# Sreyan88/audio-ssl

Measured on AMD Instinct MI355X. Metric: upstream clips/sec (1s@16kHz, 64-mel), higher is better.
Workload: dtype bf16; 1 GPU; delores-m upstream step (log-mel + 2 views + q/k conv encoders + MoCo + 3 Barlow heads + bwd + SGD), 1 s @ 16 kHz, 64 mel, batch 512/GPU, queue 65536; global_batch=512, parallelism=dp1

## Files before the change

### audio-ssl_amd/csrc/conv.hip

```cpp
#include <cstdlib>
#include "common.h"

namespace {

constexpr int CH = 64, KTOT = 576;
constexpr int WPITCH = KTOT + 8;
constexpr int PIXP = 72;
constexpr int PIXW = 96;

typedef __attribute__((address_space(3))) bf16x4* lds4_t;

struct ConvArgs {
    const bf16* X; const bf16* W; const float* bias; bf16* Y; double* sum; double* sumsq;
    int Ti, rows_total, tiles, out_f32, dbg, stat_rep;
    const float* gamma; bf16* Praw;
};

template <int FI, int PITCH, int NTH = 256>
struct Halo {
    static constexpr int TT = 256 / FI;
    static constexpr int COLS = FI + 2;
    static constexpr int ELEMS = (TT + 2) * COLS * PITCH;
    static constexpr int NV = ((TT + 2) * FI * 8 + NTH - 1) / NTH;
    static constexpr int NVEC = (TT + 2) * FI * 8;
// ... 410 lines not shown
#pragma unroll
                    for (int j = 0; j < 4; ++j) {
                        const unsigned d0 = q[0][j] ^ sm[j], d1 = q[1][j] ^ sm[j], d2 = q[2][j] ^ sm[j], d3 = q[3][j] ^ sm[j];
                        const float hi = vmax4(__builtin_bit_cast(float, d0), __builtin_bit_cast(float, d1),
                                               __builtin_bit_cast(float, d2), __builtin_bit_cast(float, d3));
                        const float lo = vmax4(__builtin_bit_cast(float, d0 << 16), __builtin_bit_cast(float, d1 << 16),
                                               __builtin_bit_cast(float, d2 << 16), __builtin_bit_cast(float, d3 << 16));
                        r[j] = __builtin_amdgcn_perm(__builtin_bit_cast(unsigned, hi), __builtin_bit_cast(unsigned, lo), 0x07060302u) ^ sm[j];
                    }
                    const unsigned odd = 0u - (unsigned)(pl & 1);
                    r = u32x4{(r[2] & odd) | (r[0] & ~odd), (r[3] & odd) | (r[1] & ~odd), (r[0] & odd) | (r[2] & ~odd), (r[1] & odd) | (r[3] & ~odd)};
                    if (a.rows_total - grow >= 2)
                        *reinterpret_cast<u32x4*>(reinterpret_cast<char*>(a.Praw) + ((grow >> 1) * (FI / 2) * 128 + po * 128 + cp * 16)) = r;
                }
            }
        }
        if (ts) ts[tsi++] = __builtin_amdgcn_s_memtime();
        asm volatile("s_waitcnt lgkmcnt(0)" ::: "memory");
        __builtin_amdgcn_s_barrier();
    }
    if (rts) rts[2] = __builtin_amdgcn_s_memrealtime();
    if (STATS) {
#pragma unroll
        for (int e = 0; e < NS; ++e) {
            float s = ssum[e], q = ssq[e];
#pragma unroll
            for (int o = 64 / NS; o < 64; o <<= 1) { s += __shfl_xor(s, o, 64); q += __shfl_xor(q, o, 64); }
            if (lane < 64 / NS) {
                const int co = lane * NS + e;
                red[(wave * 64 + co) * 2] = s; red[(wave * 64 + co) * 2 + 1] = q;
            }
        }
        __syncthreads();
        if (threadIdx.x < 128) {
            const int c = threadIdx.x >> 1, k = threadIdx.x & 1;
            double t = 0.0;
#pragma unroll
            for (int w = 0; w < 4; ++w) t += (double)red[(w * 64 + c) * 2 + k];
            const int rep = (blockIdx.x % a.stat_rep) * 128;
            atomicAdd(k == 0 ? &a.sum[rep + c] : &a.sumsq[rep + c], t);
        }
    }
}

__host__ __device__ __forceinline__ int wg_cot(int w, int n) { return n < 8 ? (n & 1) : (w & 1); }
__host__ __device__ __forceinline__ int wg_nt(int w, int n) { return n < 8 ? 4 * w + (n >> 1) : 16 + (w >> 1); }

struct WgradArgs {
    const bf16* dY; const bf16* X; float* dW; int Ti, rows_total, tiles;
    float* partial;
    int dbg;
};

template <int FI, int KG>
__global__ __launch_bounds__(256 * KG, 1) void conv3x3_wgrad_kernel(WgradArgs a) {
    using H = Halo<FI, PIXW, 256 * KG>;
    constexpr int TT = H::TT, COLS = H::COLS;
    constexpr int NTH = 256 * KG;
    constexpr int NVY = 256 * 8 / NTH;
    extern __shared__ __attribute__((aligned(16))) char smem[];
    bf16* const yl = reinterpret_cast<bf16*>(smem);
    bf16* const hl = yl + 256 * PIXW;

    const int lane = threadIdx.x & 63, wave = (threadIdx.x >> 6) & 3, grp = threadIdx.x >> 8;
    const int h = lane >> 5, half = (lane >> 4) & 1, q = (lane & 15) >> 2, p = lane & 3;
    H::zero_border(hl);

    f32x16 acc[9];
#pragma unroll
    for (int n = 0; n < 9; ++n)
#pragma unroll
        for (int r = 0; r < 16; ++r) acc[n][r] = 0.f;

    H halo;
    Vec8<bf16> ry[NVY];
    auto load_y = [&](int g0) {
#pragma unroll
        for (int i = 0; i < NVY; ++i) {
            const int v = threadIdx.x + i * NTH;
            const long pix = (long)g0 * FI + (v >> 3);
            ry[i] = pix < (long)a.rows_total * FI ? Vec8<bf16>::load(a.dY + pix * CH + (v & 7) * 8) : Vec8<bf16>::zero();
        }
    };
    auto put_y = [&]() {
#pragma unroll
        for (int i = 0; i < NVY; ++i) {
            const int v = threadIdx.x + i * NTH;
            ry[i].store(yl + (v >> 3) * PIXW + (v & 7) * 8);
        }
    };
    int tile = blockIdx.x;
    if (tile < a.tiles) { halo.load(a.X, tile * TT, a.rows_total); load_y(tile * TT); halo.put(hl); put_y(); }
    __syncthreads();

    for (; tile < a.tiles; tile += gridDim.x) {
        const int g0 = tile * TT;
        const int next = tile + gridDim.x;
        if (next < a.tiles && !(a.dbg & 2)) { halo.load(a.X, next * TT, a.rows_total); load_y(next * TT); }

#pragma unroll 1
        for (int ks = grp * (16 / KG); ks < (grp + 1) * (16 / KG) && !(a.dbg & 4); ++ks) {
            const int t_local = FI == 32 ? (ks >> 1) : ks;
            const int f0 = FI == 32 ? (ks & 1) * 16 : 0;
            const int g = g0 + t_local;
            if (g >= a.rows_total) break;
            const int ti = g % a.Ti;
            const bool okt[3] = {ti - 1 >= 0, true, ti + 1 < a.Ti};
            bf16x8 fa[2];
#pragma unroll
            for (int c2 = 0; c2 < 2; ++c2) {
                const bf16* ay = yl + (ks * 16 + 8 * h + q) * PIXW + c2 * 32 + 16 * half + 4 * p;
                const bf16x4 a0 = __builtin_amdgcn_ds_read_tr16_b64_v4bf16((lds4_t)ay);
                const bf16x4 a1 = __builtin_amdgcn_ds_read_tr16_b64_v4bf16((lds4_t)(ay + 4 * PIXW));
                fa[c2] = bf16x8{a0[0], a0[1], a0[2], a0[3], a1[0], a1[1], a1[2], a1[3]};
            }
            bf16x8 fb;
#pragma unroll
            for (int n = 0; n < 9; ++n) {
                if (n == 8 || (n & 1) == 0) {
                    const int nt = wg_nt(wave, n), tap = nt >> 1, cih = nt & 1;
                    const int dt = tap % 3, df = tap / 3;
                    const bf16* bx = hl + ((t_local + dt) * COLS + f0 + df + 8 * h + q) * PIXW + cih * 32 + 16 * half + 4 * p;
                    const bf16x4 b0 = __builtin_amdgcn_ds_read_tr16_b64_v4bf16((lds4_t)bx);
                    const bf16x4 b1 = __builtin_amdgcn_ds_read_tr16_b64_v4bf16((lds4_t)(bx + 4 * PIXW));
                    const bf16 z = (bf16)0.f;
                    fb = okt[dt] ? bf16x8{b0[0], b0[1], b0[2], b0[3], b1[0], b1[1], b1[2], b1[3]} : bf16x8{z, z, z, z, z, z, z, z};
                }
                const int c2 = wg_cot(wave, n);
                acc[n] = __builtin_amdgcn_mfma_f32_32x32x16_bf16(c2 ? fa[1] : fa[0], fb, acc[n], 0, 0, 0);
            }
        }
        __syncthreads();
        if (next < a.tiles) { halo.put(hl); put_y(); }
        __syncthreads();
    }
    if (a.partial) {
        if (KG == 2) {
            f32x4* xch = reinterpret_cast<f32x4*>(smem);
            __syncthreads();
            if (grp == 1) {
#pragma unroll
                for (int n = 0; n < 9; ++n)
#pragma unroll
                    for (int r4 = 0; r4 < 4; ++r4)
                        xch[((wave * 9 + n) * 4 + r4) * 64 + lane] = f32x4{acc[n][4 * r4], acc[n][4 * r4 + 1], acc[n][4 * r4 + 2], acc[n][4 * r4 + 3]};
            }
            __syncthreads();
            if (grp == 1) return;
            f32x4* part = reinterpret_cast<f32x4*>(a.partial + (long)blockIdx.x * (CH * KTOT));
#pragma unroll
            for (int n = 0; n < 9; ++n)
#pragma unroll
                for (int r4 = 0; r4 < 4; ++r4) {
                    const f32x4 o = xch[((wave * 9 + n) * 4 + r4) * 64 + lane];
                    part[((wave * 9 + n) * 4 + r4) * 64 + lane] = f32x4{acc[n][4 * r4] + o[0], acc[n][4 * r4 + 1] + o[1], acc[n][4 * r4 + 2] + o[2], acc[n][4 * r4 + 3] + o[3]};
                }
            return;
        }
        f32x4* part = reinterpret_cast<f32x4*>(a.partial + (long)blockIdx.x * (CH * KTOT));
#pragma unroll
        for (int n = 0; n < 9; ++n)
#pragma unroll
            for (int r4 = 0; r4 < 4; ++r4)
                part[((wave * 9 + n) * 4 + r4) * 64 + lane] = f32x4{acc[n][4 * r4], acc[n][4 * r4 + 1], acc[n][4 * r4 + 2], acc[n][4 * r4 + 3]};
        return;
    }
#pragma unroll
    for (int n = 0; n < 9; ++n) {
        const int nt = wg_nt(wave, n), tap = nt >> 1, cih = nt & 1;
        const int col = tap * 64 + cih * 32 + (lane & 31);
#pragma unroll
        for (int r = 0; r < 16; ++r) {
            const int co = wg_cot(wave, n) * 32 + (r & 3) + 8 * (r >> 2) + 4 * h;
            atomicAdd(&a.dW[co * KTOT + col], acc[n][r]);
        }
    }
}

__global__ __launch_bounds__(256) void wgrad_reduce_kernel(const float* __restrict__ partial, int nparts, float* __restrict__ dW) {
    const int i = blockIdx.x * 256 + threadIdx.x;
    if (i >= CH * KTOT) return;
    float s0 = 0.f, s1 = 0.f, s2 = 0.f, s3 = 0.f;
    int w = blockIdx.y;
    const int step = gridDim.y;
    for (; w + 3 * step < nparts; w += 4 * step) {
        s0 += partial[(long)w * (CH * KTOT) + i];
        s1 += partial[(long)(w + step) * (CH * KTOT) + i];
        s2 += partial[(long)(w + 2 * step) * (CH * KTOT) + i];
        s3 += partial[(long)(w + 3 * step) * (CH * KTOT) + i];
    }
    for (; w < nparts; w += step) s0 += partial[(long)w * (CH * KTOT) + i];
    const int e = i & 3, lane = (i >> 2) & 63, r4 = (i >> 8) & 3, wn = i >> 10;
    const int wave = wn / 9, n = wn - wave * 9;
    const int nt = wg_nt(wave, n), tap = nt >> 1, cih = nt & 1;
    const int col = tap * 64 + cih * 32 + (lane & 31);
    const int co = wg_cot(wave, n) * 32 + e + 8 * r4 + 4 * (lane >> 5);
    atomicAdd(&dW[co * KTOT + col], (s0 + s1) + (s2 + s3));
}

template <typename K>
int set_lds(K kernel, size_t bytes) {
    return hipFuncSetAttribute(reinterpret_cast<const void*>(kernel), hipFuncAttributeMaxDynamicSharedMemorySize, (int)bytes) ==
           hipSuccess ? 0 : -1;
}

}

extern "C" int audiossl_conv3x3_fwd(const void* X, const void* W, const float* bias, void* Y, int out_f32, double* sum,
                                    double* sumsq, int stat_replicas, int N, int Ti, int Fi, void* stream) {
    ASSL_REQUIRE(X && W && Y && N > 0 && Ti > 0 && (Fi == 32 || Fi == 16) && (!sum == !sumsq));
    ASSL_REQUIRE(stat_replicas >= 1 && stat_replicas <= 64 && (stat_replicas == 1 || !sum || sumsq == sum + 64));
    if (!ASSL_ALIGNED16(X) || !ASSL_ALIGNED16(W) || !ASSL_ALIGNED16(Y)) return ASSL_EALIGN;
    hipStream_t s = static_cast<hipStream_t>(stream);
#ifdef AUDIOSSL_ABLATE
    static const int conv_dbg = getenv("AUDIOSSL_CONV_DBG") ? atoi(getenv("AUDIOSSL_CONV_DBG")) : 0;
#else
    constexpr int conv_dbg = 0;
#endif
    if (sum && !(conv_dbg & 16)) {
        if (sumsq == sum + 64) {
            ASSL_ZERO(sum, sizeof(double) * 128 * stat_replicas, s);
        } else {
            ASSL_ZERO(sum, sizeof(double) * 64, s);
            ASSL_ZERO(sumsq, sizeof(double) * 64, s);
        }
    }
    const int rows = N * Ti, TT = 256 / Fi, tiles = (rows + TT - 1) / TT;
    ConvArgs a{static_cast<const bf16*>(X), static_cast<const bf16*>(W), bias, static_cast<bf16*>(Y), sum, sumsq, Ti, rows, tiles, out_f32, conv_dbg, stat_replicas};
    const int grid = tiles < 256 ? tiles : 256;
    static const int ws = getenv("AUDIOSSL_CONV_WS") ? atoi(getenv("AUDIOSSL_CONV_WS")) : 1;
    if (ws && (long)rows * Fi * 128 < 0x7FFFFF00L) {
        static bool wattr[8] = {false, false, false, false, false, false, false, false};
#define WS_LAUNCH(FI_, ST_, F32_, SLOT)                                                                    \
    do {                                                                                                  \
        const size_t lds = 2 * WsGeom<FI_>::BYTES + sizeof(float) * (64 + 4 * 64 * 2) + 4 * 64 * (F32_ ? 256 : 128) + 512; \
        if (!wattr[SLOT]) { if (set_lds(conv3x3_ws_kernel<FI_, ST_, F32_>, lds)) return ASSL_ELAUNCH; wattr[SLOT] = true; } \
        hipLaunchKernelGGL((conv3x3_ws_kernel<FI_, ST_, F32_>), dim3(grid), dim3(256), lds, s, a);       \
    } while (0)
        if (Fi == 32) {
            if (sum && !(conv_dbg & 16)) { if (out_f32) WS_LAUNCH(32, true, true, 0); else WS_LAUNCH(32, true, false, 1); }
            else     { if (out_f32) WS_LAUNCH(32, false, true, 2); else WS_LAUNCH(32, false, false, 3); }
        } else {
            if (sum) { if (out_f32) WS_LAUNCH(16, true, true, 4); else WS_LAUNCH(16, true, false, 5); }
            else     { if (out_f32) WS_LAUNCH(16, false, true, 6); else WS_LAUNCH(16, false, false, 7); }
        }
#undef WS_LAUNCH
        ASSL_LAUNCH_CHECK();
    }
    static const int nw = getenv("AUDIOSSL_CONV_WAVES") ? atoi(getenv("AUDIOSSL_CONV_WAVES")) : 8;
    static bool attr[4] = {false, false, false, false};
#define CONV_LAUNCH(FI_, NW_, SLOT)                                                                       \
    do {                                                                                                  \
        const size_t lds = sizeof(bf16) * (CH * WPITCH + Halo<FI_, PIXP>::ELEMS);                         \
        if (!attr[SLOT]) { if (set_lds(conv3x3_kernel<FI_, NW_>, lds)) return ASSL_ELAUNCH; attr[SLOT] = true; } \
        hipLaunchKernelGGL((conv3x3_kernel<FI_, NW_>), dim3(grid), dim3(64 * NW_), lds, s, a);           \
    } while (0)
    if (Fi == 32) { if (nw == 8) CONV_LAUNCH(32, 8, 0); else CONV_LAUNCH(32, 4, 1); }
    else          { if (nw == 8) CONV_LAUNCH(16, 8, 2); else CONV_LAUNCH(16, 4, 3); }
#undef CONV_LAUNCH
    ASSL_LAUNCH_CHECK();
}

extern "C" int audiossl_conv3x3_pool_fwd(const void* X, const void* W, const float* bias, const float* gamma, void* Y, void* Praw,
                                         double* sum, double* sumsq, int stat_replicas, int N, int Ti, int Fi, void* stream) {
    ASSL_REQUIRE(X && W && gamma && Praw && sum && sumsq && N > 0 && Ti > 0 && (Ti % 2) == 0 && (Fi == 32 || Fi == 16));
    ASSL_REQUIRE(stat_replicas >= 1 && stat_replicas <= 64 && (stat_replicas == 1 || sumsq == sum + 64));
    const int rows = N * Ti, TT = 256 / Fi, tiles = (rows + TT - 1) / TT;
    ASSL_REQUIRE((long)rows * Fi * 128 < 0x7FFFFF00L);
    if (!ASSL_ALIGNED16(X) || !ASSL_ALIGNED16(W) || !ASSL_ALIGNED16(Y) || !ASSL_ALIGNED16(Praw)) return ASSL_EALIGN;
    hipStream_t s = static_cast<hipStream_t>(stream);
    if (sumsq == sum + 64) {
        ASSL_ZERO(sum, sizeof(double) * 128 * stat_replicas, s);
    } else {
        ASSL_ZERO(sum, sizeof(double) * 64, s);
        ASSL_ZERO(sumsq, sizeof(double) * 64, s);
    }
    ConvArgs a{static_cast<const bf16*>(X), static_cast<const bf16*>(W), bias, static_cast<bf16*>(Y), sum, sumsq, Ti, rows, tiles, 0, 0,
               stat_replicas, gamma, static_cast<bf16*>(Praw)};
    const int grid = tiles < 256 ? tiles : 256;
    static bool pattr[4] = {false, false, false, false};
#define POOL_LAUNCH(FI_, KEEP_, SLOT)                                                                     \
    do {                                                                                                  \
        const size_t lds = 2 * WsGeom<FI_>::BYTES + sizeof(float) * (64 + 4 * 64 * 2) + 4 * 64 * 128 + 512 + 256; \
        if (!pattr[SLOT]) { if (set_lds(conv3x3_ws_kernel<FI_, true, false, 2, true, KEEP_>, lds)) return ASSL_ELAUNCH; pattr[SLOT] = true; } \
        hipLaunchKernelGGL((conv3x3_ws_kernel<FI_, true, false, 2, true, KEEP_>), dim3(grid), dim3(256), lds, s, a); \
    } while (0)
    if (Fi == 32) { if (Y) POOL_LAUNCH(32, true, 0); else POOL_LAUNCH(32, false, 1); }
    else          { if (Y) POOL_LAUNCH(16, true, 2); else POOL_LAUNCH(16, false, 3); }
#undef POOL_LAUNCH
    ASSL_LAUNCH_CHECK();
}

extern "C" int audiossl_conv3x3_wgrad(const void* dY, const void* X, float* dWp, float* workspace, long workspace_floats, int N,
                                      int Ti, int Fi, void* stream) {
    ASSL_REQUIRE(dY && X && dWp && N > 0 && Ti > 0 && (Fi == 32 || Fi == 16));
    if (!ASSL_ALIGNED16(X) || !ASSL_ALIGNED16(dY)) return ASSL_EALIGN;
    hipStream_t s = static_cast<hipStream_t>(stream);
    const int rows = N * Ti, TT = 256 / Fi, tiles = (rows + TT - 1) / TT;
    const int grid = tiles < 256 ? tiles : 256;
    const bool two_stage = workspace != nullptr && workspace_floats >= (long)grid * CH * KTOT;
#ifdef AUDIOSSL_ABLATE
    static const int wg_dbg = getenv("AUDIOSSL_CONV_DBG") ? atoi(getenv("AUDIOSSL_CONV_DBG")) : 0;
#else
    constexpr int wg_dbg = 0;
#endif
    WgradArgs a{static_cast<const bf16*>(dY), static_cast<const bf16*>(X), dWp, Ti, rows, tiles, two_stage ? workspace : nullptr, wg_dbg};
    static const int kg_env = getenv("AUDIOSSL_WGRAD_KG") ? atoi(getenv("AUDIOSSL_WGRAD_KG")) : 0;
    const int kg = kg_env ? kg_env : (two_stage ? 2 : 1);
    static bool attr[4] = {false, false, false, false};
#define WGRAD_LAUNCH(FI_, KG_, SLOT)                                                                      \
    do {                                                                                                  \
        const size_t lds = max(sizeof(bf16) * (256 * PIXW + Halo<FI_, PIXW>::ELEMS), (size_t)(KG_ == 2 ? 4 * 9 * 16 * 64 * 4 : 0)); \
        if (!attr[SLOT]) { if (set_lds(conv3x3_wgrad_kernel<FI_, KG_>, lds)) return ASSL_ELAUNCH; attr[SLOT] = true; } \
        hipLaunchKernelGGL((conv3x3_wgrad_kernel<FI_, KG_>), dim3(grid), dim3(256 * KG_), lds, s, a);    \
    } while (0)
    if (Fi == 32) { if (kg == 2) WGRAD_LAUNCH(32, 2, 0); else WGRAD_LAUNCH(32, 1, 1); }
    else          { if (kg == 2) WGRAD_LAUNCH(16, 2, 2); else WGRAD_LAUNCH(16, 1, 3); }
#undef WGRAD_LAUNCH
    if (two_stage)
        hipLaunchKernelGGL(wgrad_reduce_kernel, dim3(CH * KTOT / 256, 8), dim3(256), 0, s, workspace, grid, dWp);
    ASSL_LAUNCH_CHECK();
}
```

### audio-ssl_amd/src/engine.py

```python
import os

import torch

from src import _native as N

import os as _os
_STEM_VALU = _os.environ.get("AUDIOSSL_STEM_VALU") == "1"
BN_MOMENTUM = 0.1
BN_EPS = 1e-5
_BN_FUSED = _os.environ.get("AUDIOSSL_BN_FUSED", "1") != "0"


ONE_STREAM = os.environ.get("AUDIOSSL_ONE_STREAM", "0") == "1"


_CAPTURE_ORIGIN = []


class capture_scope:

    def __enter__(self):
        _CAPTURE_ORIGIN.append(torch.cuda.current_stream())
        return self

# ... 411 lines not shown
        N.call("tmean3_fwd", dtype, o32, None if x1_fused else c.P1, x1, x1_parts, T1, F1, c.P2, x2, T2, F2, c.P3, x3, T3, F3, Nimg)
    d = P["fc.0.weight"].shape[0]
    kin = F3 * 64
    M = Nimg * T3
    c.d, c.kin, c.M = d, kin, M
    if before_fc is not None:
        before_fc()
    if Wc is not None:
        c.fw1, c.fw2 = Wc["fc.0.weight"], Wc["fc.3.weight"]
    else:
        c.fw1, c.fw2 = cast(dtype, P["fc.0.weight"]), cast(dtype, P["fc.3.weight"])
    if keep is not None and not isinstance(keep, torch.Tensor) and (dtype != N.BF16 or not train):
        keep = keep.materialise()
    c.keep = keep if train else None
    scale = 1.0 / (1.0 - p_drop) if c.keep is not None else 1.0
    if c.keep is not None and not isinstance(c.keep, torch.Tensor):
        vk = c.keep
        c.H1 = torch.empty(M, d, dtype=torch.bfloat16, device=c.P3.device)
        N.call("gemm_dropout", 0, 0, M, d, kin, 1.0, c.P3, kin, c.fw1, kin, c.H1, d, P["fc.0.bias"], 1, vk.seed, float(vk.p), vk.counter,
               float(scale))
    else:
        c.H1 = linear_fwd(dtype, c.P3, c.fw1, M, d, kin, bias=P["fc.0.bias"], relu=1, keep=c.keep, keep_scale=scale)
    c.H2 = linear_fwd(dtype, c.H1, c.fw2, M, d, d, bias=P["fc.3.bias"], relu=1)
    return x1, x2, x3, c.H2.view(Nimg, T3, d), c


def ragged_pool(dtype, H, lens, hop=160, shift=3, want_mean=True, want_maxmean=True):
    Nimg, Tt, D = H.shape
    mean = _empty((Nimg, D), torch.float32, like=H) if want_mean else None
    mm = _empty((Nimg, D), torch.float32, like=H) if want_maxmean else None
    N.call("meanmax_ragged_fwd", dtype, H.contiguous(), mean, mm, lens, hop, shift, Nimg, Tt, D)
    return mean, mm


def _conv_block_bwd(dtype, Y, dP, dxl, st, Nimg, Ti, Fi, Pin, Wd, G_w, G_gamma, G_beta, need_dx, col, keep, dx_bf16=False, Pout=None):
    td = N.torch_dtype(dtype)
    scale, shift, mean, rstd = st
    M = Nimg * Ti * Fi
    dY = torch.empty((M, 64), dtype=td, device=Y.device)
    stat = ARENA.scratch((33 * 128,), torch.float32, Y)
    yd = N.F32 if Y.dtype == torch.float32 else dtype
    if SYNC_BN is None and Pout is not None and _BN_STATS_P and Pout.dtype == td:
        N.call("bn_relu_pool_bwd_p", dtype, yd, GD, Y, Pout, dP, dxl, scale, shift, mean, rstd, stat, dY, G_gamma, G_beta, Nimg, Ti, Fi)
    elif SYNC_BN is None:
        N.call("bn_relu_pool_bwd", dtype, yd, GD, Y, dP, dxl, scale, shift, mean, rstd, stat, dY, G_gamma, G_beta, Nimg, Ti, Fi)
    else:
        N.call("bn_relu_pool_bwd_stats", dtype, yd, GD, Y, dP, dxl, scale, shift, mean, rstd, stat, Nimg, Ti, Fi)
        gstat = SYNC_BN.all_reduce(stat[:128].clone())
        N.call("bn_relu_pool_bwd_apply", dtype, yd, GD, Y, dP, dxl, scale, shift, mean, rstd, stat, gstat, float(M * SYNC_BN.world), dY,
               G_gamma, G_beta, Nimg, Ti, Fi)
    fused = dtype == N.BF16 and Fi in (16, 32)
    if fused:
        def wg():
            dWp = ARENA.zeros((64, 576), torch.float32, device=Y.device)
            ws = _wgrad_workspace(Y.device)
            N.call("conv3x3_wgrad", dY, Pin, dWp, ws, ws.numel(), Nimg, Ti, Fi)
            N.call("unpack_conv_dw", dWp, G_w)
            return dWp
        keep.append((dY, WGRAD.run(Y.device, wg)))
    else:
        dWp = ARENA.zeros((64, 576), torch.float32, device=Y.device)
        N.call("im2col3x3", dtype, Pin, col, Nimg, Ti, Fi)
        gemm(dtype, 1, 1, 64, 576, M, dY, 64, col, 576, dWp, 576, out_f32=1, atomic=1, ksplit=_ksplit(64, 576, M, 1024))
        N.call("unpack_conv_dw", dWp, G_w)
    if not need_dx:
        return None
    dx_bf16 = dx_bf16 and fused
    dPin = _empty((Nimg, Ti, Fi, 64), torch.bfloat16 if dx_bf16 else torch.float32, like=Y)
    if fused:
        N.call("conv3x3_fwd", dY, Wd, None, dPin, 0 if dx_bf16 else 1, None, None, 1, Nimg, Ti, Fi)
    else:
        N.call("im2col3x3", dtype, dY, col, Nimg, Ti, Fi)
        gemm(dtype, 0, 0, M, 64, 576, col, 576, Wd, 576, dPin, 64)
    return dPin


def encoder_backward(c, G, dA2=None, dH2=None, dx1=None, dx2=None, dx3=None, dx_late=None, grads_zero=False):
    dtype, Nimg, M, d, kin = c.dtype, c.N, c.M, c.d, c.kin
    T1, F1, T2, F2, T3, F3 = c.dims
    td = N.torch_dtype(dtype)
    assert c.train, "backward needs a train-mode forward (batch statistics)"
    assert c.need_bwd, "this forward ran with need_bwd=False: the conv outputs were not kept"
    if dA2 is None:
        dA2 = _empty((M, d), td, like=c.H2)
        N.call("relu_bwd", dtype, dH2.contiguous(), c.H2, dA2, M * d)
    dev = c.H2.device
    def w2():
        linear_bwd_w(dtype, dA2, c.H1, G["fc.3.weight"], M, d, d, dw_zero=grads_zero)
        colsum_add(dtype, dA2, M, d, G["fc.3.bias"])
    WGRAD.run(dev, w2)
    scale = 1.0 / (1.0 - c.p_drop) if c.keep is not None else 1.0
    dA1 = linear_bwd_x(dtype, dA2, c.fw2, M, d, d, alpha=scale, gate=c.H1)
    def w1():
        linear_bwd_w(dtype, dA1, c.P3, G["fc.0.weight"], M, d, kin, dw_zero=grads_zero)
        colsum_add(dtype, dA1, M, d, G["fc.0.bias"])
    WGRAD.run(dev, w1)
    dP3 = linear_bwd_x(dtype, dA1, c.fw1, M, d, kin, out_f32=1)
    if dx_late is not None:
        dx1, dx2, dx3 = dx_late()
    col = _col_buffer(dtype, Nimg, T1, F1, c.H2)
    keep = []
    dP2 = _conv_block_bwd(dtype, c.Y3, dP3, dx3, c.st3, Nimg, T2, F2, c.P2, c.W3d, G["features_3.0.weight"],
                          G["features_3.1.weight"], G["features_3.1.bias"], True, col, keep, Pout=c.P3)
    dP1 = _conv_block_bwd(dtype, c.Y2, dP2, dx2, c.st2, Nimg, T1, F1, c.P1, c.W2d, G["features_2.0.weight"],
                          G["features_2.1.weight"], G["features_2.1.bias"], True, col, keep, dx_bf16=bool(c.stem_mfma) and _DP1_BF16,
                          Pout=c.P2)
    gd1 = N.BF16 if dP1.dtype == torch.bfloat16 else GD
    acc = ARENA.scratch((32 * 64 * 11,), torch.float32, c.H2)
    P = c.P
    w1, b1, g1 = P["features_1.0.weight"].reshape(64, 9), P["features_1.0.bias"], P["features_1.1.weight"]
    gw, gb = G["features_1.0.weight"].view(64, 9), G["features_1.0.bias"]
# ... 361 lines not shown
```

### include/audiossl_hip.h

```cpp
#ifndef AUDIOSSL_HIP_H
#define AUDIOSSL_HIP_H

#include <stdint.h>

#ifdef __cplusplus
extern "C" {
#endif

#define AUDIOSSL_OK 0
#define AUDIOSSL_EINVAL (-1)
#define AUDIOSSL_ELAUNCH (-2)
#define AUDIOSSL_EALIGN (-3)

int audiossl_logmel_fwd(const float* wave, float* out, int B, int L, int T, int n_fft, int hop, int n_mels, int taps,
                        const float* win, const float* tw, const float* melw, const int* mel_start, float eps_pow,
                        float eps_log, int apply_log, void* stream);
int audiossl_logmel_ragged_fwd(const float* wave, const int* lens, const int* lens_host, float* out, int B, int Lmax, int Tmax,
                               int n_fft, int hop, int n_mels, int taps, const float* win, const float* tw, const float* melw,
                               const int* mel_start, float eps_pow, float eps_log, int apply_log, void* stream);

int audiossl_fbank_fwd(const float* wave, const int* lens, const int* partner, const float* lam, float* clip_mean,
                       const int* bands, const int* bands_host, float* out, int B, int Lmax, int win_len, int shift, int n_fft, int n_mels,
                       int taps, int T_target, const float* win, const float* tw, const float* melw, const int* mel_start,
                       float preemph, float eps_log, float mean, float std, int skip_norm, int time_major, void* stream);
// ... 51 lines not shown
int audiossl_bn_relu_pool_train_fwd(int dtype, int ydtype, const void* Y, const double* sum, const double* sumsq, int stat_replicas,
                                    double count, const float* gamma, const float* beta, float* running_mean, float* running_var,
                                    float momentum, float eps, void* P, float* scale, float* shift, float* save_mean, float* save_rstd,
                                    int N, int Ti, int Fi, void* stream);
int audiossl_bn_relu_pooled_fwd(int dtype, const void* Praw, const float* scale, const float* shift, void* P, int N, int To, int Fo,
                                void* stream);
int audiossl_bn_relu_pooled_train_fwd(int dtype, const void* Praw, const double* sum, const double* sumsq, int stat_replicas,
                                      double count, const float* gamma, const float* beta, float* running_mean, float* running_var,
                                      float momentum, float eps, void* P, float* scale, float* shift, float* save_mean,
                                      float* save_rstd, int N, int To, int Fo, void* stream);
int audiossl_tmean_fwd(int dtype, int out_f32, const void* P, void* xl, int N, int To, int Fo, void* stream);
int audiossl_tmean3_fwd(int dtype, int out_f32, const void* P1, void* x1, const float* x1_parts, int To1, int Fo1, const void* P2,
                        void* x2, int To2, int Fo2, const void* P3, void* x3, int To3, int Fo3, int N, void* stream);
int audiossl_bn_relu_pool_bwd(int dtype, int ydtype, int gdtype, const void* Y, const void* dP, const void* dxl, const float* scale,
                              const float* shift, const float* mean, const float* rstd, float* stat, void* dY,
                              float* dgamma, float* dbeta, int N, int Ti, int Fi, void* stream);
int audiossl_bn_relu_pool_bwd_p(int dtype, int ydtype, int gdtype, const void* Y, const void* P, const void* dP, const void* dxl,
                                const float* scale, const float* shift, const float* mean, const float* rstd, float* stat, void* dY,
                                float* dgamma, float* dbeta, int N, int Ti, int Fi, void* stream);
int audiossl_conv1_moments(const float* img, int N, int F, int T, double* mom, void* stream);
int audiossl_conv1_finalize(double* mom_totals, const float* w, const float* bias, const float* gamma, const float* beta,
                            float* running_mean, float* running_var, float momentum, float eps, double count, float* scale,
                            float* shift, float* save_mean, float* save_rstd, void* stream);
int audiossl_conv1_bwd_sums(int dtype, int conv_dtype, const float* img, int N, int F, int T, const float* w, const float* bias,
                            const float* gamma, const float* scale, const float* shift, const float* mean, const float* rstd,
                            const double* mom, const void* dP, const void* dxl, float* acc, float* lstat, void* stream);
int audiossl_conv1_bwd_finalize(const float* acc, const double* mom, const float* w, const float* bias, const float* gamma,
                                const float* mean, const float* rstd, double count_global, const float* gstat, float* dW,
                                float* dbias, float* dgamma, float* dbeta, void* stream);
int audiossl_bn_relu_pool_bwd_stats(int dtype, int ydtype, int gdtype, const void* Y, const void* dP, const void* dxl,
                                    const float* scale, const float* shift, const float* mean, const float* rstd, float* stat,
                                    int N, int Ti, int Fi, void* stream);
int audiossl_bn_relu_pool_bwd_apply(int dtype, int ydtype, int gdtype, const void* Y, const void* dP, const void* dxl,
                                    const float* scale, const float* shift, const float* mean, const float* rstd, float* stat,
                                    const float* gstat, double count_global, void* dY, float* dgamma, float* dbeta, int N, int Ti,
                                    int Fi, void* stream);
int audiossl_colbn_bwd_stats(int dtype, int adtype, int gdtype, const void* a, const void* dh, const float* scale,
                             const float* shift, const float* mean, const float* rstd, int relu, int groups, long M, int C,
                             double* tmp, void* stream);
int audiossl_colbn_bwd_apply(int dtype, int adtype, int gdtype, const void* a, const void* dh, const float* scale,
                             const float* shift, const float* mean, const float* rstd, int relu, int groups, long M, int C,
                             const double* sums, double count, void* da, void* stream);
int audiossl_im2col3x3(int dtype, const void* X, void* col, int N, int Ti, int Fi, void* stream);
int audiossl_pack_conv_w(int dtype, const float* W, void* Wf, void* Wd, void* stream);
int audiossl_pack_conv_w2(int dtype, const float* Wa, void* Wfa, void* Wda, const float* Wb, void* Wfb, void* Wdb, void* stream);
int audiossl_unpack_conv_dw(const float* dWp, float* dW, void* stream);

int audiossl_conv3x3_fwd(const void* X, const void* W, const float* bias, void* Y, int out_f32, double* sum,
                         double* sumsq, int stat_replicas, int N, int Ti, int Fi, void* stream);
int audiossl_conv3x3_pool_fwd(const void* X, const void* W, const float* bias, const float* gamma, void* Y, void* Praw, double* sum,
                              double* sumsq, int stat_replicas, int N, int Ti, int Fi, void* stream);
int audiossl_conv3x3_wgrad(const void* dY, const void* X, float* dWp, float* workspace, long workspace_floats, int N, int Ti,
                           int Fi, void* stream);

int audiossl_gemm(int dtype, int trans_a, int trans_b, int M, int N, int K, float alpha, const void* A, long lda,
                  const void* B, long ldb, void* C, long ldc, const float* bias, int relu, const uint8_t* keep, long ldk,
                  float keep_scale, const void* gate, long ldg, int out_f32, int atomic, int ksplit, const float* resid,
                  long ldr, void* stream);

int audiossl_gemm_dropout(int trans_a, int trans_b, int M, int N, int K, float alpha, const void* A, long lda, const void* B,
                          long ldb, void* C, long ldc, const float* bias, int relu, unsigned long long seed, float p,
                          const long long* counter, float keep_scale, void* stream);

int audiossl_gemm_multi(int count, int trans_a, int trans_b, int M, const int* N, const int* K, float alpha,
                        const void* const* A, const long* lda, const void* const* B, const long* ldb, void* const* C,
                        const long* ldc, int out_f32, int atomic, int ksplit, void* stream);
int audiossl_gemm_multi_sgd(int count, int trans_a, int trans_b, int M, const int* Nv, const int* K, float alpha,
                            const void* const* A, const long* lda, const void* const* B, const long* ldb, float* const* P,
                            float* const* Mom, void* const* Shadow, const long* ldp, float lr, float momentum, float weight_decay,
                            float grad_scale, const float* grad_scale_dev, void* stream);
int audiossl_gemm_multi_barlow(int count, int D, const int* K, float alpha, const void* const* A, const long* lda,
                               const void* const* B, const long* ldb, void* const* dc, const float* coef, const float* dscale,
                               float* const* loss_rep, void* stream);

int audiossl_maxmean_fwd(int dtype, int out_f32, const void* H, void* y, uint8_t* arg, int N, int Tt, int D, void* stream);
int audiossl_maxmean_bwd(int dtype, int gdtype, const void* dy, const uint8_t* arg, const void* H, void* dA, int N, int Tt,
                         int D, void* stream);

int audiossl_tail_mask(int dtype, void* P, const int* lens, int hop, int shift, int N, int To, long row_elems, void* stream);
int audiossl_tmean3_ragged_fwd(int dtype, const void* P1, float* x1, int To1, int Fo1, const void* P2, float* x2, int To2, int Fo2,
                               const void* P3, float* x3, int To3, int Fo3, const int* lens, int hop, int N, void* stream);
int audiossl_meanmax_ragged_fwd(int dtype, const void* H, float* mean, float* maxmean, const int* lens, int hop, int shift, int N,
                                int Tt, int D, void* stream);

int audiossl_colbn_fwd(int dtype, int adtype, const void* a, const float* scale, const float* shift, int relu, void* h,
                       int groups, long M, int C, void* stream);
int audiossl_colbn_train_fwd(int dtype, int adtype, const void* a, const float* gamma, const float* beta,
                             float* running_mean, float* running_var, float momentum, float eps, int relu, int groups,
                             long M, int C, void* h, float* scale, float* shift, float* save_mean, float* save_rstd,
                             void* stream);
int audiossl_colbn_bwd(int dtype, int adtype, int gdtype, const void* a, const void* dh, const float* scale, const float* shift, const float* mean,
                       const float* rstd, int relu, int groups, long M, int C, double* tmp, void* da, float* dgamma,
                       float* dbeta, void* stream);
int audiossl_colbn_train_fwd_multi(int count, int adtype, const void* const* a, const float* const* gamma,
                                   const float* const* beta, float* const* running_mean, float* const* running_var,
                                   float momentum, float eps, int relu, int groups, long M, int C, void* const* h,
                                   float* const* stats, void* stream);
int audiossl_colbn_bwd_multi(int count, int adtype, int gdtype, const void* const* a, const void* const* dh,
                             const float* const* stats, int relu, int groups, long M, int C, void* const* da,
                             float* const* dgamma, float* const* dbeta, void* stream);
int audiossl_barlow_loss_multi(int count, const float* const* c, int D, const float* coef, const float* dscale,
                               void* const* dc, float* const* loss_out, void* stream);
int audiossl_add_d2f(const double* src, float* dst, int n, void* stream);
int audiossl_barlow_loss(int dtype, const float* c, int D, float coef, float dscale, void* dc, float* loss_out,
                         void* stream);

// ... 140 lines not shown
```

Baseline: 267,000 clips/s.

## Add DMA double-buffered LDS loads to conv wgrad and fuse dW unpack

Adds a wgrad kernel variant that loads X halo and dY tiles straight into double-buffered, XOR-swizzled LDS with buffer_load...lds. This removes the register round-trip and lets the next tile's loads overlap compute. The inner loop is software-pipelined, prefetching the next k-step's fragments while the current MFMAs run. The reduce kernel can now write dW directly in parameter layout, so the separate zero/unpack pass disappears. Risks: this relies on inline asm touching m0, uses twice the LDS, and the param path assumes the two-stage workspace exists.

Result: no change. 268,700 clips/s, median of 6 (+0.7%).

```diff
diff --git a/audio-ssl_amd/csrc/conv.hip b/audio-ssl_amd/csrc/conv.hip
--- a/audio-ssl_amd/csrc/conv.hip
+++ b/audio-ssl_amd/csrc/conv.hip
@@ -486,19 +486,11 @@
     int dbg;
 };
 
-template <int FI, int KG>
+template <int FI, int KG, bool DMA = false>
 __global__ __launch_bounds__(256 * KG, 1) void conv3x3_wgrad_kernel(WgradArgs a) {
-    using H = Halo<FI, PIXW, 256 * KG>;
-    constexpr int TT = H::TT, COLS = H::COLS;
-    constexpr int NTH = 256 * KG;
-    constexpr int NVY = 256 * 8 / NTH;
     extern __shared__ __attribute__((aligned(16))) char smem[];
-    bf16* const yl = reinterpret_cast<bf16*>(smem);
-    bf16* const hl = yl + 256 * PIXW;
-
     const int lane = threadIdx.x & 63, wave = (threadIdx.x >> 6) & 3, grp = threadIdx.x >> 8;
     const int h = lane >> 5, half = (lane >> 4) & 1, q = (lane & 15) >> 2, p = lane & 3;
-    H::zero_border(hl);
 
     f32x16 acc[9];
 #pragma unroll
@@ -506,67 +498,203 @@
 #pragma unroll
         for (int r = 0; r < 16; ++r) acc[n][r] = 0.f;
 
-    H halo;
-    Vec8<bf16> ry[NVY];
-    auto load_y = [&](int g0) {
-#pragma unroll
-        for (int i = 0; i < NVY; ++i) {
-            const int v = threadIdx.x + i * NTH;
-            const long pix = (long)g0 * FI + (v >> 3);
-            ry[i] = pix < (long)a.rows_total * FI ? Vec8<bf16>::load(a.dY + pix * CH + (v & 7) * 8) : Vec8<bf16>::zero();
-        }
-    };
-    auto put_y = [&]() {
-#pragma unroll
-        for (int i = 0; i < NVY; ++i) {
-            const int v = threadIdx.x + i * NTH;
-            ry[i].store(yl + (v >> 3) * PIXW + (v & 7) * 8);
-        }
-    };
-    int tile = blockIdx.x;
-    if (tile < a.tiles) { halo.load(a.X, tile * TT, a.rows_total); load_y(tile * TT); halo.put(hl); put_y(); }
-    __syncthreads();
-
-    for (; tile < a.tiles; tile += gridDim.x) {
-        const int g0 = tile * TT;
-        const int next = tile + gridDim.x;
-        if (next < a.tiles && !(a.dbg & 2)) { halo.load(a.X, next * TT, a.rows_total); load_y(next * TT); }
+    if constexpr (!DMA) {
+        using H = Halo<FI, PIXW, 256 * KG>;
+        constexpr int TT = H::TT, COLS = H::COLS;
+        constexpr int NTH = 256 * KG;
+        constexpr int NVY = 256 * 8 / NTH;
+        bf16* const yl = reinterpret_cast<bf16*>(smem);
+        bf16* const hl = yl + 256 * PIXW;
+        H::zero_border(hl);
+
+        H halo;
+        Vec8<bf16> ry[NVY];
+        auto load_y = [&](int g0) {
+#pragma unroll
+            for (int i = 0; i < NVY; ++i) {
+                const int v = threadIdx.x + i * NTH;
+                const long pix = (long)g0 * FI + (v >> 3);
+                ry[i] = pix < (long)a.rows_total * FI ? Vec8<bf16>::load(a.dY + pix * CH + (v & 7) * 8) : Vec8<bf16>::zero();
+            }
+        };
+        auto put_y = [&]() {
+#pragma unroll
+            for (int i = 0; i < NVY; ++i) {
+                const int v = threadIdx.x + i * NTH;
+                ry[i].store(yl + (v >> 3) * PIXW + (v & 7) * 8);
+            }
+        };
+        int tile = blockIdx.x;
+        if (tile < a.tiles) { halo.load(a.X, tile * TT, a.rows_total); load_y(tile * TT); halo.put(hl); put_y(); }
+        __syncthreads();
+
+        for (; tile < a.tiles; tile += gridDim.x) {
+            const int g0 = tile * TT;
+            const int next = tile + gridDim.x;
+            if (next < a.tiles && !(a.dbg & 2)) { halo.load(a.X, next * TT, a.rows_total); load_y(next * TT); }
 
 #pragma unroll 1
-        for (int ks = grp * (16 / KG); ks < (grp + 1) * (16 / KG) && !(a.dbg & 4); ++ks) {
-            const int t_local = FI == 32 ? (ks >> 1) : ks;
-            const int f0 = FI == 32 ? (ks & 1) * 16 : 0;
-            const int g = g0 + t_local;
-            if (g >= a.rows_total) break;
-            const int ti = g % a.Ti;
-            const bool okt[3] = {ti - 1 >= 0, true, ti + 1 < a.Ti};
-            bf16x8 fa[2];
-#pragma unroll
-            for (int c2 = 0; c2 < 2; ++c2) {
-                const bf16* ay = yl + (ks * 16 + 8 * h + q) * PIXW + c2 * 32 + 16 * half + 4 * p;
-                const bf16x4 a0 = __builtin_amdgcn_ds_read_tr16_b64_v4bf16((lds4_t)ay);
-                const bf16x4 a1 = __builtin_amdgcn_ds_read_tr16_b64_v4bf16((lds4_t)(ay + 4 * PIXW));
-                fa[c2] = bf16x8{a0[0], a0[1], a0[2], a0[3], a1[0], a1[1], a1[2], a1[3]};
-            }
-            bf16x8 fb;
-#pragma unroll
-            for (int n = 0; n < 9; ++n) {
-                if (n == 8 || (n & 1) == 0) {
-                    const int nt = wg_nt(wave, n), tap = nt >> 1, cih = nt & 1;
-                    const int dt = tap % 3, df = tap / 3;
-                    const bf16* bx = hl + ((t_local + dt) * COLS + f0 + df + 8 * h + q) * PIXW + cih * 32 + 16 * half + 4 * p;
-                    const bf16x4 b0 = __builtin_amdgcn_ds_read_tr16_b64_v4bf16((lds4_t)bx);
-                    const bf16x4 b1 = __builtin_amdgcn_ds_read_tr16_b64_v4bf16((lds4_t)(bx + 4 * PIXW));
-                    const bf16 z = (bf16)0.f;
-                    fb = okt[dt] ? bf16x8{b0[0], b0[1], b0[2], b0[3], b1[0], b1[1], b1[2], b1[3]} : bf16x8{z, z, z, z, z, z, z, z};
+            for (int ks = grp * (16 / KG); ks < (grp + 1) * (16 / KG) && !(a.dbg & 4); ++ks) {
+                const int t_local = FI == 32 ? (ks >> 1) : ks;
+                const int f0 = FI == 32 ? (ks & 1) * 16 : 0;
+                const int g = g0 + t_local;
+                if (g >= a.rows_total) break;
+                const int ti = g % a.Ti;
+                const bool okt[3] = {ti - 1 >= 0, true, ti + 1 < a.Ti};
+                bf16x8 fa[2];
+#pragma unroll
+                for (int c2 = 0; c2 < 2; ++c2) {
+                    const bf16* ay = yl + (ks * 16 + 8 * h + q) * PIXW + c2 * 32 + 16 * half + 4 * p;
+                    const bf16x4 a0 = __builtin_amdgcn_ds_read_tr16_b64_v4bf16((lds4_t)ay);
+                    const bf16x4 a1 = __builtin_amdgcn_ds_read_tr16_b64_v4bf16((lds4_t)(ay + 4 * PIXW));
+                    fa[c2] = bf16x8{a0[0], a0[1], a0[2], a0[3], a1[0], a1[1], a1[2], a1[3]};
                 }
-                const int c2 = wg_cot(wave, n);
-                acc[n] = __builtin_amdgcn_mfma_f32_32x32x16_bf16(c2 ? fa[1] : fa[0], fb, acc[n], 0, 0, 0);
-            }
-        }
-        __syncthreads();
-        if (next < a.tiles) { halo.put(hl); put_y(); }
-        __syncthreads();
+                bf16x8 fb;
+#pragma unroll
+                for (int n = 0; n < 9; ++n) {
+                    if (n == 8 || (n & 1) == 0) {
+                        const int nt = wg_nt(wave, n), tap = nt >> 1, cih = nt & 1;
+                        const int dt = tap % 3, df = tap / 3;
+                        const bf16* bx = hl + ((t_local + dt) * COLS + f0 + df + 8 * h + q) * PIXW + cih * 32 + 16 * half + 4 * p;
+                        const bf16x4 b0 = __builtin_amdgcn_ds_read_tr16_b64_v4bf16((lds4_t)bx);
+                        const bf16x4 b1 = __builtin_amdgcn_ds_read_tr16_b64_v4bf16((lds4_t)(bx + 4 * PIXW));
+                        const bf16 z = (bf16)0.f;
+                        fb = okt[dt] ? bf16x8{b0[0], b0[1], b0[2], b0[3], b1[0], b1[1], b1[2], b1[3]} : bf16x8{z, z, z, z, z, z, z, z};
+                    }
+                    const int c2 = wg_cot(wave, n);
+                    acc[n] = __builtin_amdgcn_mfma_f32_32x32x16_bf16(c2 ? fa[1] : fa[0], fb, acc[n], 0, 0, 0);
+                }
+            }
+            __syncthreads();
+            if (next < a.tiles) { halo.put(hl); put_y(); }
+            __syncthreads();
+        }
+    } else {
+        using G = WsGeom<FI>;
+        constexpr int TT = G::TT, COLS = G::COLS, NW = 4 * KG;
+        constexpr int SET = G::BYTES + 256 * 128;
+        constexpr int XPW = (G::UNITS + NW - 1) / NW, YPW = 32 / NW;
+        typedef __attribute__((address_space(3))) void* lptr_t;
+
+        const int wv = __builtin_amdgcn_readfirstlane(threadIdx.x >> 6);
+        for (int i = threadIdx.x; i < 2 * G::ROWS * 2 * 8; i += 256 * KG) {
+            const int b = i / (G::ROWS * 16), r = (i / 16) % G::ROWS, side = (i >> 3) & 1, c8 = i & 7;
+            *reinterpret_cast<f32x4*>(smem + b * SET + (r * COLS + side * (FI + 1)) * 128 + c8 * 16) = f32x4{0.f, 0.f, 0.f, 0.f};
+        }
+
+        const unsigned nbytes = (unsigned)((long)a.rows_total * FI * 128);
+        const unsigned long xb = reinterpret_cast<unsigned long>(a.X), yb = reinterpret_cast<unsigned long>(a.dY);
+        const u32x4 rx = {(unsigned)xb, (unsigned)(xb >> 32) & 0xFFFFu, nbytes, 0x00020000u};
+        const u32x4 ry = {(unsigned)yb, (unsigned)(yb >> 32) & 0xFFFFu, nbytes, 0x00020000u};
+        auto dma16 = [](const u32x4& rsrc, unsigned lds, unsigned voff) {
+            unsigned keep;
+            asm volatile("s_mov_b32 %0, m0\n\ts_mov_b32 m0, %3\n\ts_nop 4\n\tbuffer_load_dwordx4 %1, %2, 0 offen lds\n\ts_mov_b32 m0, %0"
+                         : "=&s"(keep) : "v"(voff), "s"(rsrc), "s"(lds) : "memory");
+        };
+        const unsigned lds0 = (unsigned)(size_t)((lptr_t)smem);
+        const int pl = lane >> 3, cp = lane & 7;
+        const unsigned vx = pl * 128 + ((cp ^ ((((1 + pl) >> 1) & 1) << 2)) << 4);
+        const unsigned vy = pl * 128 + ((cp ^ (((pl >> 1) & 1) << 2)) << 4);
+        auto dma_tile = [&](int g0, unsigned set) {
+#pragma unroll
+            for (int i = 0; i < XPW; ++i) {
+                const int u = wv + NW * i;
+                if (u < G::UNITS) {
+                    const int row = u / G::SEGS, seg = u % G::SEGS;
+                    const int gr = g0 - 1 + row;
+                    const unsigned so = (gr >= 0 && gr < a.rows_total) ? (unsigned)(gr * FI + 8 * seg) * 128u : 0x7FFFFF00u;
+                    dma16(rx, set + (row * COLS + 1 + 8 * seg) * 128, vx + so);
+                }
+            }
+#pragma unroll
+            for (int i = 0; i < YPW; ++i) {
+                const int u = wv + NW * i;
+                const unsigned so = (unsigned)(g0 * FI + 8 * u) * 128u;
+                dma16(ry, set + G::BYTES + u * 1024, vy + so);
+            }
+        };
+
+        const int lo = 32 * half + 8 * p;
+        const int yo = (8 * h + q) * 128 + lo, yk = (q >> 1) & 1;
+        int xo[5], xdt[5];
+#pragma unroll
+        for (int j = 0; j < 5; ++j) {
+            const int nt = wg_nt(wave, j < 4 ? 2 * j : 8), tap = nt >> 1, cih = nt & 1;
+            const int dt = tap % 3, df = tap / 3;
+            xo[j] = (dt * COLS + df + 8 * h + q) * 128 + (cih ^ (((df + q) >> 1) & 1)) * 64 + lo;
+            xdt[j] = dt;
+        }
+        auto frag = [](int addr) {
+            const bf16x4 r0 = __builtin_amdgcn_ds_read_tr16_b64_v4bf16((lds4_t)(size_t)addr);
+            const bf16x4 r1 = __builtin_amdgcn_ds_read_tr16_b64_v4bf16((lds4_t)(size_t)(addr + 4 * 128));
+            return bf16x8{r0[0], r0[1], r0[2], r0[3], r1[0], r1[1], r1[2], r1[3]};
+        };
+
+        int tile = blockIdx.x, cur = 0;
+        if (tile < a.tiles) dma_tile(tile * TT, lds0);
+        asm volatile("s_waitcnt vmcnt(0) lgkmcnt(0)" ::: "memory");
+        __builtin_amdgcn_s_barrier();
+
+        for (; tile < a.tiles; tile += gridDim.x, cur ^= 1) {
+            const int g0 = tile * TT;
+            const int next = tile + gridDim.x;
+            if (next < a.tiles && !(a.dbg & 2)) dma_tile(next * TT, lds0 + (cur ^ 1) * SET);
+            const int hl = lds0 + cur * SET;
+            const int yl = hl + G::BYTES;
+
+            const int rows_in = min(TT, a.rows_total - g0);
+            const int kb = grp * (16 / KG);
+            const int ke = (a.dbg & 4) ? kb : min((grp + 1) * (16 / KG), rows_in * (FI == 32 ? 2 : 1));
+            auto okt_of = [&](int ks, bool& o0, bool& o2) {
+                const int ti = (g0 + (FI == 32 ? (ks >> 1) : ks)) % a.Ti;
+                o0 = ti - 1 >= 0; o2 = ti + 1 < a.Ti;
+            };
+            auto rd_a = [&](int ks, int c2) { return frag(yl + ks * 16 * 128 + yo + (c2 ^ yk) * 64); };
+            auto rd_b = [&](int ks, int j) {
+                const int t_local = FI == 32 ? (ks >> 1) : ks, f0 = FI == 32 ? (ks & 1) * 16 : 0;
+                return frag(hl + (t_local * COLS + f0) * 128 + xo[j]);
+            };
+            auto sel = [&](const bf16x8& v, int j, bool o0, bool o2) {
+                const bf16 z = (bf16)0.f;
+                const bool ok = xdt[j] == 0 ? o0 : (xdt[j] == 2 ? o2 : true);
+                return ok ? v : bf16x8{z, z, z, z, z, z, z, z};
+            };
+            if (kb < ke) {
+                bf16x8 fa[2], fb[5];
+                bool o0, o2;
+                okt_of(kb, o0, o2);
+                fa[0] = rd_a(kb, 0); fa[1] = rd_a(kb, 1);
+#pragma unroll
+                for (int j = 0; j < 5; ++j) fb[j] = rd_b(kb, j);
+#pragma unroll 1
+                for (int ks = kb; ks < ke; ++ks) {
+                    const int kn = min(ks + 1, ke - 1);
+                    bf16x8 na[2], nb[5];
+                    bool n0, n2;
+                    okt_of(kn, n0, n2);
+#pragma unroll
+                    for (int j = 0; j < 5; ++j) {
+                        const bf16x8 f = sel(fb[j], j, o0, o2);
+                        __builtin_amdgcn_sched_barrier(0);
+                        if (j < 4) {
+                            acc[2 * j] = __builtin_amdgcn_mfma_f32_32x32x16_bf16(fa[0], f, acc[2 * j], 0, 0, 0);
+                            acc[2 * j + 1] = __builtin_amdgcn_mfma_f32_32x32x16_bf16(fa[1], f, acc[2 * j + 1], 0, 0, 0);
+                        } else {
+                            acc[8] = __builtin_amdgcn_mfma_f32_32x32x16_bf16(wg_cot(wave, 8) ? fa[1] : fa[0], f, acc[8], 0, 0, 0);
+                        }
+                        __builtin_amdgcn_sched_barrier(0);
+                        nb[j] = rd_b(kn, j);
+                        if (j == 0) { na[0] = rd_a(kn, 0); na[1] = rd_a(kn, 1); }
+                    }
+                    fa[0] = na[0]; fa[1] = na[1];
+#pragma unroll
+                    for (int j = 0; j < 5; ++j) fb[j] = nb[j];
+                    o0 = n0; o2 = n2;
+                }
+            }
+            asm volatile("s_waitcnt vmcnt(0) lgkmcnt(0)" ::: "memory");
+            __builtin_amdgcn_s_barrier();
+        }
     }
     if (a.partial) {
         if (KG == 2) {
@@ -611,6 +739,7 @@
     }
 }
 
+template <bool PARAM>
 __global__ __launch_bounds__(256) void wgrad_reduce_kernel(const float* __restrict__ partial, int nparts, float* __restrict__ dW) {
     const int i = blockIdx.x * 256 + threadIdx.x;
     if (i >= CH * KTOT) return;
@@ -629,7 +758,7 @@
     const int nt = wg_nt(wave, n), tap = nt >> 1, cih = nt & 1;
     const int col = tap * 64 + cih * 32 + (lane & 31);
     const int co = wg_cot(wave, n) * 32 + e + 8 * r4 + 4 * (lane >> 5);
-    atomicAdd(&dW[co * KTOT + col], (s0 + s1) + (s2 + s3));
+    atomicAdd(&dW[PARAM ? (co * 64 + cih * 32 + (lane & 31)) * 9 + tap : co * KTOT + col], (s0 + s1) + (s2 + s3));
 }
 
 template <typename K>
@@ -725,14 +854,15 @@
     ASSL_LAUNCH_CHECK();
 }
 
-extern "C" int audiossl_conv3x3_wgrad(const void* dY, const void* X, float* dWp, float* workspace, long workspace_floats, int N,
-                                      int Ti, int Fi, void* stream) {
+static int wgrad_launch(const void* dY, const void* X, float* dWp, float* workspace, long workspace_floats, int N, int Ti, int Fi,
+                        void* stream, bool param) {
     ASSL_REQUIRE(dY && X && dWp && N > 0 && Ti > 0 && (Fi == 32 || Fi == 16));
     if (!ASSL_ALIGNED16(X) || !ASSL_ALIGNED16(dY)) return ASSL_EALIGN;
     hipStream_t s = static_cast<hipStream_t>(stream);
     const int rows = N * Ti, TT = 256 / Fi, tiles = (rows + TT - 1) / TT;
     const int grid = tiles < 256 ? tiles : 256;
     const bool two_stage = workspace != nullptr && workspace_floats >= (long)grid * CH * KTOT;
+    ASSL_REQUIRE(two_stage || !param);
 #ifdef AUDIOSSL_ABLATE
     static const int wg_dbg = getenv("AUDIOSSL_CONV_DBG") ? atoi(getenv("AUDIOSSL_CONV_DBG")) : 0;
 #else
@@ -741,17 +871,37 @@
     WgradArgs a{static_cast<const bf16*>(dY), static_cast<const bf16*>(X), dWp, Ti, rows, tiles, two_stage ? workspace : nullptr, wg_dbg};
     static const int kg_env = getenv("AUDIOSSL_WGRAD_KG") ? atoi(getenv("AUDIOSSL_WGRAD_KG")) : 0;
     const int kg = kg_env ? kg_env : (two_stage ? 2 : 1);
-    static bool attr[4] = {false, false, false, false};
-#define WGRAD_LAUNCH(FI_, KG_, SLOT)                                                                      \
+    static const int dma_env = getenv("AUDIOSSL_WGRAD_DMA") ? atoi(getenv("AUDIOSSL_WGRAD_DMA")) : 1;
+    const bool dma = dma_env && (long)rows * Fi * 128 < 0x7FFFFF00L;
+    static bool attr[8] = {false, false, false, false, false, false, false, false};
+#define WGRAD_LAUNCH(FI_, KG_, DMA_, SLOT)                                                                \
     do {                                                                                                  \
-        const size_t lds = max(sizeof(bf16) * (256 * PIXW + Halo<FI_, PIXW>::ELEMS), (size_t)(KG_ == 2 ? 4 * 9 * 16 * 64 * 4 : 0)); \
-        if (!attr[SLOT]) { if (set_lds(conv3x3_wgrad_kernel<FI_, KG_>, lds)) return ASSL_ELAUNCH; attr[SLOT] = true; } \
-        hipLaunchKernelGGL((conv3x3_wgrad_kernel<FI_, KG_>), dim3(grid), dim3(256 * KG_), lds, s, a);    \
+        const size_t tiles_lds = DMA_ ? 2 * (size_t)(WsGeom<FI_>::BYTES + 256 * 128) : sizeof(bf16) * (256 * PIXW + Halo<FI_, PIXW>::ELEMS); \
+        const size_t lds = max(tiles_lds, (size_t)(KG_ == 2 ? 4 * 9 * 16 * 64 * 4 : 0));                  \
+        if (!attr[SLOT]) { if (set_lds(conv3x3_wgrad_kernel<FI_, KG_, DMA_>, lds)) return ASSL_ELAUNCH; attr[SLOT] = true; } \
+        hipLaunchKernelGGL((conv3x3_wgrad_kernel<FI_, KG_, DMA_>), dim3(grid), dim3(256 * KG_), lds, s, a); \
     } while (0)
-    if (Fi == 32) { if (kg == 2) WGRAD_LAUNCH(32, 2, 0); else WGRAD_LAUNCH(32, 1, 1); }
-    else          { if (kg == 2) WGRAD_LAUNCH(16, 2, 2); else WGRAD_LAUNCH(16, 1, 3); }
+    if (dma) {
+        if (Fi == 32) { if (kg == 2) WGRAD_LAUNCH(32, 2, true, 4); else WGRAD_LAUNCH(32, 1, true, 5); }
+        else          { if (kg == 2) WGRAD_LAUNCH(16, 2, true, 6); else WGRAD_LAUNCH(16, 1, true, 7); }
+    } else {
+        if (Fi == 32) { if (kg == 2) WGRAD_LAUNCH(32, 2, false, 0); else WGRAD_LAUNCH(32, 1, false, 1); }
+        else          { if (kg == 2) WGRAD_LAUNCH(16, 2, false, 2); else WGRAD_LAUNCH(16, 1, false, 3); }
+    }
 #undef WGRAD_LAUNCH
-    if (two_stage)
-        hipLaunchKernelGGL(wgrad_reduce_kernel, dim3(CH * KTOT / 256, 8), dim3(256), 0, s, workspace, grid, dWp);
+    if (two_stage) {
+        if (param) hipLaunchKernelGGL(wgrad_reduce_kernel<true>, dim3(CH * KTOT / 256, 8), dim3(256), 0, s, workspace, grid, dWp);
+        else hipLaunchKernelGGL(wgrad_reduce_kernel<false>, dim3(CH * KTOT / 256, 8), dim3(256), 0, s, workspace, grid, dWp);
+    }
     ASSL_LAUNCH_CHECK();
 }
+
+extern "C" int audiossl_conv3x3_wgrad(const void* dY, const void* X, float* dWp, float* workspace, long workspace_floats, int N,
+                                      int Ti, int Fi, void* stream) {
+    return wgrad_launch(dY, X, dWp, workspace, workspace_floats, N, Ti, Fi, stream, false);
+}
+
+extern "C" int audiossl_conv3x3_wgrad_param(const void* dY, const void* X, float* dW, float* workspace, long workspace_floats, int N,
+                                            int Ti, int Fi, void* stream) {
+    return wgrad_launch(dY, X, dW, workspace, workspace_floats, N, Ti, Fi, stream, true);
+}
diff --git a/audio-ssl_amd/src/engine.py b/audio-ssl_amd/src/engine.py
--- a/audio-ssl_amd/src/engine.py
+++ b/audio-ssl_amd/src/engine.py
@@ -487,11 +487,8 @@
     fused = dtype == N.BF16 and Fi in (16, 32)
     if fused:
         def wg():
-            dWp = ARENA.zeros((64, 576), torch.float32, device=Y.device)
             ws = _wgrad_workspace(Y.device)
-            N.call("conv3x3_wgrad", dY, Pin, dWp, ws, ws.numel(), Nimg, Ti, Fi)
-            N.call("unpack_conv_dw", dWp, G_w)
-            return dWp
+            N.call("conv3x3_wgrad_param", dY, Pin, G_w, ws, ws.numel(), Nimg, Ti, Fi)
         keep.append((dY, WGRAD.run(Y.device, wg)))
     else:
         dWp = ARENA.zeros((64, 576), torch.float32, device=Y.device)
diff --git a/include/audiossl_hip.h b/include/audiossl_hip.h
--- a/include/audiossl_hip.h
+++ b/include/audiossl_hip.h
@@ -127,6 +127,8 @@
                               double* sumsq, int stat_replicas, int N, int Ti, int Fi, void* stream);
 int audiossl_conv3x3_wgrad(const void* dY, const void* X, float* dWp, float* workspace, long workspace_floats, int N, int Ti,
                            int Fi, void* stream);
+int audiossl_conv3x3_wgrad_param(const void* dY, const void* X, float* dW, float* workspace, long workspace_floats, int N, int Ti,
+                                 int Fi, void* stream);
 
 int audiossl_gemm(int dtype, int trans_a, int trans_b, int M, int N, int K, float alpha, const void* A, long lda,
                   const void* B, long ldb, void* C, long ldc, const float* bias, int relu, const uint8_t* keep, long ldk,
```
